# vliu15/speech-masters-thesis

Measured on AMD Instinct MI355X. Metric: LJSpeech utterances/sec per VQ-VAE train step, higher is better.
Workload: dtype bf16

## Files before the change

### speech-masters-thesis_amd/csrc/conv_wgrad.hip

```cpp
#include <algorithm>
#include <cstdlib>

#include "conv_common.h"

namespace smt {

struct WgradArgs {
  const void* x; const void* dy; float* slab;
  const int* lens_in;
  long long x_bs, dy_bs;
  int ldx, ldy;
  int B, Tin, Tout, Ty, Cin, Cout;
  int taps, stride, dil, pad, out_stride, out_offset;
  int rows_per_chunk, chunks_per_batch, nblk_ci, nblk_co, with_bias;
};

template <typename T> struct WTr;
template <> struct WTr<__bf16> {
  static constexpr int R = 128;
  static constexpr int pitch(int ch) { return ch + 32; }
};
template <> struct WTr<float> {
  static constexpr int R = 64;
  static constexpr int pitch(int ch) { return ch + 4; }
};

__device__ __forceinline__ int tr_lane_row(int lane) { return 8 * (lane >> 5) + ((lane & 15) >> 2); }
__device__ __forceinline__ int tr_lane_col(int lane) { return 16 * ((lane >> 4) & 1) + 4 * (lane & 3); }
__device__ __forceinline__ bf16x8 tr_read2(const void* a0, int step4_bytes) {
  const unsigned char* a = reinterpret_cast<const unsigned char*>(a0);
  return lds_tr2(a, a + step4_bytes);
}
__device__ __forceinline__ bf16x8 frag_tr_bf16(const __bf16* tile, int pitch, int row0, int col0, int lane) {
  return tr_read2(tile + (row0 + tr_lane_row(lane)) * pitch + col0 + tr_lane_col(lane), 4 * pitch * 2);
}

struct WgBlock { int nblk, blk, cgl; };
__device__ __forceinline__ WgBlock wgrad_block(int nblk_ci, int nblk_co) {
  WgBlock w;
  w.nblk = nblk_ci * nblk_co;
  const int xcd = blockIdx.x & 7, q = blockIdx.x >> 3;
  w.blk = q % w.nblk;
  w.cgl = (q / w.nblk) * 8 + xcd;
  return w;
}

template <typename T, int NT, int CIB, bool STRIDED>
__global__ __launch_bounds__(CIB * 4) void conv_wgrad_kernel(WgradArgs p) {
  constexpr int EPV = Tr<T>::EPV;
  constexpr int R = WTr<T>::R;
  constexpr int CB = 64;
  constexpr int WNC = CIB / 32;
  constexpr int NTHR = 128 * WNC;
  constexpr int PITCH_DY = WTr<T>::pitch(CB), PITCH_X = WTr<T>::pitch(CIB);
  extern __shared__ __attribute__((aligned(16))) unsigned char smem[];
  const int tid = threadIdx.x, lane = tid & 63, wave = tid >> 6;
  const int wm = wave / WNC, wn = wave % WNC;
  const int r = lane & 31, hh = lane >> 5;

  const WgBlock w = wgrad_block(p.nblk_ci, p.nblk_co);
  if (w.cgl >= p.B * p.chunks_per_batch) return;
  const int co0 = (w.blk / p.nblk_ci) * CB, ci0 = (w.blk % p.nblk_ci) * CIB;
  const int b = w.cgl / p.chunks_per_batch;
  const int chunk = w.cgl % p.chunks_per_batch;
  const int t_begin = chunk * p.rows_per_chunk;
  const int t_end = min(p.Tout, t_begin + p.rows_per_chunk);

  const int rows_x = (R - 1) * p.stride + (p.taps - 1) * p.dil + 1;
  T* lds_dy = reinterpret_cast<T*>(smem);
  T* lds_x = lds_dy + R * PITCH_DY;
  const T* xg = reinterpret_cast<const T*>(p.x) + (long long)b * p.x_bs;
  const T* dyg = reinterpret_cast<const T*>(p.dy) + (long long)b * p.dy_bs;
  const int len_in = p.lens_in ? min(p.lens_in[b], p.Tin) : p.Tin;
  const bool bias_plane = p.with_bias && (ci0 == 0);
  const int ntaps = p.taps;

  f32x16 acc[NT];
#pragma unroll
  for (int j = 0; j < NT; ++j)
#pragma unroll
    for (int e = 0; e < 16; ++e) acc[j][e] = 0.f;

  for (int t0 = t_begin; t0 < t_end; t0 += R) {
    __syncthreads();
    constexpr int VPR_DY = CB / EPV, VPR_X = CIB / EPV;
    constexpr int UB = (NT > 6) ? 4 : 8;
    const int tin0 = t0 * p.stride - p.pad;
    const int n_dy = R * VPR_DY, n_x = rows_x * VPR_X;
    for (int f0 = tid; f0 < n_dy + n_x; f0 += NTHR * UB) {
      Vec<T, EPV> v[UB];
#pragma unroll
      for (int u = 0; u < UB; ++u) {
        const int f = f0 + NTHR * u;
#pragma unroll
        for (int e = 0; e < EPV; ++e) v[u].v[e] = (T)0.f;
        if (f < n_dy) {
          const int row = f / VPR_DY, cv = f % VPR_DY;
          const int t = t0 + row;
          const int ty = t * p.out_stride + p.out_offset;
          if (t < t_end && ty < p.Ty && co0 + cv * EPV < p.Cout)
            v[u] = *reinterpret_cast<const Vec<T, EPV>*>(dyg + (long long)ty * p.ldy + co0 + cv * EPV);
        } else if (f < n_dy + n_x) {
          const int g = f - n_dy;
          const int row = g / VPR_X, cv = g % VPR_X;
          const int tin = tin0 + row;
          if (tin >= 0 && tin < len_in && ci0 + cv * EPV < p.Cin)
            v[u] = *reinterpret_cast<const Vec<T, EPV>*>(xg + (long long)tin * p.ldx + ci0 + cv * EPV);
        }
      }
#pragma unroll
      for (int u = 0; u < UB; ++u) {
        const int f = f0 + NTHR * u;
        if (f < n_dy) {
          *reinterpret_cast<Vec<T, EPV>*>(lds_dy + (f / VPR_DY) * PITCH_DY + (f % VPR_DY) * EPV) = v[u];
        } else if (f < n_dy + n_x) {
          const int g = f - n_dy;
          *reinterpret_cast<Vec<T, EPV>*>(lds_x + (g / VPR_X) * PITCH_X + (g % VPR_X) * EPV) = v[u];
        }
      }
    }
    __syncthreads();

    if constexpr (sizeof(T) == 2) {
      const __bf16* dyt = reinterpret_cast<const __bf16*>(lds_dy);
      const __bf16* xt = reinterpret_cast<const __bf16*>(lds_x);
      bf16x8 ones;
#pragma unroll
      for (int e = 0; e < 8; ++e) ones[e] = (__bf16)1.0f;
#pragma unroll 1
      for (int k0 = 0; k0 < R; k0 += 16) {
        bf16x8 a = frag_tr_bf16(dyt, PITCH_DY, k0, wm * 32, lane);
#pragma unroll
        for (int j = 0; j < NT; ++j) {
          if (j < ntaps) {
            bf16x8 bfrag;
            if constexpr (!STRIDED) {
              bfrag = frag_tr_bf16(xt, PITCH_X, k0 + j * p.dil, wn * 32, lane);
            } else {
              typedef short s16x8 __attribute__((ext_vector_type(8)));
              s16x8 tmp;
#pragma unroll
              for (int e = 0; e < 8; ++e) {
                const short* sp = reinterpret_cast<const short*>(xt) +
                                  ((k0 + 8 * hh + e) * p.stride + j * p.dil) * PITCH_X + wn * 32 + r;
                tmp[e] = *sp;
              }
              bfrag = __builtin_bit_cast(bf16x8, tmp);
            }
            acc[j] = __builtin_amdgcn_mfma_f32_32x32x16_bf16(a, bfrag, acc[j], 0, 0, 0);
          } else if (j == ntaps && bias_plane) {
            acc[j] = __builtin_amdgcn_mfma_f32_32x32x16_bf16(a, ones, acc[j], 0, 0, 0);
          }
        }
      }
    } else {
      const float* dyt = reinterpret_cast<const float*>(lds_dy);
      const float* xt = reinterpret_cast<const float*>(lds_x);
#pragma unroll 2
      for (int k0 = 0; k0 < R; k0 += 2) {
        const float a = dyt[(k0 + hh) * PITCH_DY + wm * 32 + r];
#pragma unroll
        for (int j = 0; j < NT; ++j) {
          if (j < ntaps) {
            const float bv = xt[((k0 + hh) * p.stride + j * p.dil) * PITCH_X + wn * 32 + r];
            acc[j] = __builtin_amdgcn_mfma_f32_32x32x2f32(a, bv, acc[j], 0, 0, 0);
          } else if (j == ntaps && bias_plane) {
            acc[j] = __builtin_amdgcn_mfma_f32_32x32x2f32(a, 1.0f, acc[j], 0, 0, 0);
          }
        }
      }
    }
  }
  const int planes = ntaps + 1;
  float* out = p.slab + ((size_t)w.cgl * w.nblk + w.blk) * (size_t)planes * CB * CIB;
#pragma unroll
  for (int j = 0; j < NT; ++j) {
    if (j >= planes) break;
#pragma unroll
    for (int e = 0; e < 16; ++e) {
      const int row = wm * 32 + (e & 3) + 8 * (e >> 2) + 4 * hh;
      const int col = wn * 32 + r;
      out[((size_t)j * CB + row) * CIB + col] = acc[j][e];
    }
  }
}

__device__ __forceinline__ int swz_dy(int row) { return ((row >> 1) & 1) << 2; }
__device__ __forceinline__ int swz_x(int row) { return (row & 3) << 2; }
__device__ __forceinline__ int swz_col_bytes(int col, int swz) { return (((col >> 3) ^ swz) << 4) + (col & 7) * 2; }

template <int NT>
__global__ __launch_bounds__(512) void conv_wgrad_dma_kernel(WgradArgs p) {
  typedef __bf16 T;
  constexpr int R = 128, CB = 64, CIB = 128, WNC = 4, NTHR = 512;
  constexpr int DYB = CB * 2, XB = CIB * 2;
  constexpr int DY_BYTES = R * DYB;
  extern __shared__ __attribute__((aligned(16))) unsigned char smem[];
  const int tid = threadIdx.x, lane = tid & 63, wave = tid >> 6;
  const int wm = wave / WNC, wn = wave % WNC;
  const int r = lane & 31, hh = lane >> 5;

  const WgBlock w = wgrad_block(p.nblk_ci, p.nblk_co);
  if (w.cgl >= p.B * p.chunks_per_batch) return;
  const int co0 = (w.blk / p.nblk_ci) * CB, ci0 = (w.blk % p.nblk_ci) * CIB;
  const int b = w.cgl / p.chunks_per_batch;
  const int chunk = w.cgl % p.chunks_per_batch;
  const int t_begin = chunk * p.rows_per_chunk;
  const int t_end = min(p.Tout, t_begin + p.rows_per_chunk);

  const int rows_x = (R - 1) + (p.taps - 1) * p.dil + 1;
  const int rows_x_pad = (rows_x + 3) & ~3;
  const size_t buf_bytes = (size_t)DY_BYTES + (size_t)rows_x_pad * XB;
  const T* xg = reinterpret_cast<const T*>(p.x) + (long long)b * p.x_bs;
  const T* dyg = reinterpret_cast<const T*>(p.dy) + (long long)b * p.dy_bs;
  const int len_in = max(0, p.lens_in ? min(p.lens_in[b], p.Tin) : p.Tin);
  const bool bias_plane = p.with_bias && (ci0 == 0);
  const int ntaps = p.taps;

  f32x16 acc[NT];
#pragma unroll
  for (int j = 0; j < NT; ++j)
#pragma unroll
    for (int e = 0; e < 16; ++e) acc[j][e] = 0.f;

  const UntrackedRsrc rdy = untracked_rsrc(dyg + co0, 0, (unsigned)min((long long)0xfffffff0ll, (long long)p.Tout * p.ldy * 2));
  const UntrackedRsrc rxx = untracked_rsrc(xg + ci0, 0, (unsigned)min((long long)0xfffffff0ll, (long long)len_in * p.ldx * 2));
  const unsigned pdy = (unsigned)(p.ldy * 2), pxx = (unsigned)(p.ldx * 2);
  auto stage = [&](int t0, int buf) {
    unsigned char* base = smem + (size_t)buf * buf_bytes;
    for (int g = wave; g < R / 8; g += NTHR / 64) {
      const int row = 8 * g + (lane >> 3), pos = lane & 7;
      const int t = t0 + row;
      const int ch = pos ^ swz_dy(row);
      untracked_dma16(rdy, t < t_end ? (unsigned)t * pdy + (unsigned)(ch << 4) : 0xffffff00u, base + g * 1024);
    }
    const int tin0 = t0 - p.pad;
    for (int g = wave; g < rows_x_pad / 4; g += NTHR / 64) {
      const int row = 4 * g + (lane >> 4), pos = lane & 15;
      const int ch = pos ^ swz_x(row);
      const int tin = tin0 + row;
      const bool ok = (row < rows_x) && (tin >= 0) && (tin < len_in);
      untracked_dma16(rxx, ok ? (unsigned)tin * pxx + (unsigned)(ch << 4) : 0xffffff00u, base + DY_BYTES + g * 1024);
    }
  };

  bf16x8 ones;
#pragma unroll
  for (int e = 0; e < 8; ++e) ones[e] = (__bf16)1.0f;

  const int lrow = tr_lane_row(lane);
  const int coly = wm * 32 + tr_lane_col(lane), colx = wn * 32 + tr_lane_col(lane);
  const int dyoff = lrow * DYB + swz_col_bytes(coly, swz_dy(lrow));
  int xoff[NT];
#pragma unroll
  for (int j = 0; j < NT; ++j) {
    const int rj = lrow + j * p.dil;
    xoff[j] = rj * XB + swz_col_bytes(colx, swz_x(rj));
  }

  stage(t_begin, 0);
  vm_wait<0>();
  int buf = 0;
  for (int t0 = t_begin; t0 < t_end; t0 += R, buf ^= 1) {
    lgkm_wait<0>();
    __builtin_amdgcn_s_barrier();
    if (t0 + R < t_end) stage(t0 + R, buf ^ 1);
    const unsigned char* dyt = smem + (size_t)buf * buf_bytes + dyoff;
    const unsigned char* xbase = smem + (size_t)buf * buf_bytes + DY_BYTES;
#pragma unroll
    for (int k0 = 0; k0 < R; k0 += 16) {
      const bf16x8 a = tr_read2(dyt + k0 * DYB, 4 * DYB);
#pragma unroll
      for (int j = 0; j < NT; ++j) {
        if (j < ntaps) {
          const bf16x8 bfrag = tr_read2(xbase + xoff[j] + k0 * XB, 4 * XB);
          acc[j] = __builtin_amdgcn_mfma_f32_32x32x16_bf16(a, bfrag, acc[j], 0, 0, 0);
        } else if (j == ntaps && bias_plane) {
          acc[j] = __builtin_amdgcn_mfma_f32_32x32x16_bf16(a, ones, acc[j], 0, 0, 0);
        }
      }
    }
    step_end_wait<0>();
  }
  const int planes = ntaps + 1;
  float* out = p.slab + ((size_t)w.cgl * w.nblk + w.blk) * (size_t)planes * CB * CIB;
#pragma unroll
  for (int j = 0; j < NT; ++j) {
    if (j >= planes) break;
#pragma unroll
    for (int e = 0; e < 16; ++e) {
      const int row = wm * 32 + (e & 3) + 8 * (e >> 2) + 4 * hh;
      const int col = wn * 32 + r;
      out[((size_t)j * CB + row) * CIB + col] = acc[j][e];
    }
  }
}

struct ShiftArgs {
  const void* x; const void* dy; float* slab; const int* lens_in;
  long long x_bs, dy_bs;
  int ldx, ldy;
  int B, Tin, Tout, pad, rs;
  int tiles_per_item, tiles_per_wg, n_chunks, nblk_ci, nblk_co, with_bias;
};

#ifndef SMT_WGRAD_STAMP
#define SMT_WGRAD_STAMP 0
#endif
#if SMT_WGRAD_STAMP
__device__ unsigned long long wg_dbg[256 * 8 * 8];
__device__ __forceinline__ unsigned long long wg_stamp() {
  unsigned long long t;
  __builtin_amdgcn_sched_barrier(0);
  asm volatile("s_memtime %0\n\ts_waitcnt lgkmcnt(0)" : "=s"(t) : : "memory");
  __builtin_amdgcn_sched_barrier(0);
  return t;
}
#define WG_SUMS unsigned long long wg_sum[5] = {0, 0, 0, 0, 0}
#define WG_T(var) const unsigned long long var = wg_stamp()
#define WG_ACC(k, a, b) wg_sum[k] += (b) - (a)
#define WG_DUMP do { if (lane == 0 && blockIdx.x < 256) for (int k_ = 0; k_ < 5; ++k_) wg_dbg[(blockIdx.x * 8 + wave) * 8 + k_] += wg_sum[k_]; } while (0)
#else
#define WG_SUMS do {} while (0)
#define WG_T(var) do {} while (0)
#define WG_ACC(k, a, b) do {} while (0)
#define WG_DUMP do {} while (0)
#endif

constexpr int SH_R = 128, SH_XROWS = SH_R + 8, SH_DY = SH_R * 128, SH_X = SH_XROWS * 256, SH_STAGE = SH_DY + SH_X;

template <int NTAPS>
__global__ __launch_bounds__(512) void conv_wgrad_shift_kernel(ShiftArgs p, const __bf16* __restrict__ zero_page) {
  constexpr int CB = 64, CIB = 128, WNC = 4, DYB = CB * 2, XB = CIB * 2, PLANES = NTAPS + 1;
  extern __shared__ __attribute__((aligned(16))) unsigned char smem[];
  const int tid = threadIdx.x, lane = tid & 63;
  const int wave = __builtin_amdgcn_readfirstlane(tid >> 6);
  const int wm = wave / WNC, wn = wave % WNC;
  const int r = lane & 31, hh = lane >> 5;

  const WgBlock w = wgrad_block(p.nblk_ci, p.nblk_co);
  if (w.cgl >= p.n_chunks) return;
  const int co0 = (w.blk / p.nblk_ci) * CB, ci0 = (w.blk % p.nblk_ci) * CIB;
  const int ntiles = p.tiles_per_item * p.B * p.rs;
  const int tile_begin = w.cgl * p.tiles_per_wg;
  const int tile_end = min(ntiles, tile_begin + p.tiles_per_wg);
  const int rs = p.rs;
  const bool bias_plane = p.with_bias && (ci0 == 0);

  f32x16 acc[PLANES];
#pragma unroll
  for (int j = 0; j < PLANES; ++j)
#pragma unroll
    for (int e = 0; e < 16; ++e) acc[j][e] = 0.f;

  constexpr int SH_PIECES = 7;
  constexpr int SH_PPS = 2;
  static_assert(SH_PPS <= NTAPS && SH_PPS * (SH_R / 16) >= SH_PIECES, "the pieces fit the k-loop");
  const unsigned pdy = (unsigned)p.ldy * rs * 2u, pxx = (unsigned)p.ldx * rs * 2u;
  const int dyrow = 8 * wave + (lane >> 3), xrow = 4 * wave + (lane >> 4);
  const unsigned voff_dy = (unsigned)dyrow * pdy + (unsigned)(((lane & 7) ^ swz_dy(dyrow)) << 4);
  const unsigned voff_x = (unsigned)xrow * pxx + (unsigned)(((lane & 15) ^ swz_x(xrow)) << 4);
  const unsigned voff_x6 = (128 + xrow < SH_R + NTAPS - 1) ? voff_x + 128u * pxx : 0x80000000u;
  struct Src { __amdgpu_buffer_rsrc_t rdy, rxx; unsigned sdy, sx; };
  auto item_source = [&](int item, Src& s) {
    const int b = item / rs, cls = item - b * rs;
    const int Tc = (p.Tout - cls + rs - 1) / rs;
    const int len_full = p.lens_in ? min(scalar_load_i32(p.lens_in + b), p.Tin) : p.Tin;
    const int len_in = max(0, (len_full - cls + rs - 1) / rs);
    s.rdy = ws_rsrc(p.dy, ((long long)b * p.dy_bs + (long long)cls * p.ldy + co0) * 2, (unsigned)Tc * pdy);
    s.rxx = ws_rsrc(p.x, ((long long)b * p.x_bs + (long long)cls * p.ldx + ci0) * 2, (unsigned)len_in * pxx);
  };
  auto tile_source = [&](int t0, Src& s) {
    s.sdy = (unsigned)t0 * pdy;
    s.sx = (unsigned)(t0 - p.pad) * pxx;
  };
  auto piece = [&](const Src& s, int i, int buf) {
    unsigned char* base = smem + (size_t)buf * SH_STAGE;
    if (i < 2) ws_dma16(s.rdy, voff_dy + s.sdy + (unsigned)(64 * i) * pdy, base + (wave + 8 * i) * 1024);
    else if (i < 6) ws_dma16(s.rxx, voff_x + s.sx + (unsigned)(32 * (i - 2)) * pxx, base + SH_DY + (wave + 8 * (i - 2)) * 1024);
    else if (wave < 2) ws_dma16(s.rxx, voff_x6 + s.sx, base + SH_DY + (wave + 32) * 1024);
  };

  bf16x8 ones;
#pragma unroll
  for (int e = 0; e < 8; ++e) ones[e] = (__bf16)1.0f;

  const int tg = lane >> 4, tq = (lane & 15) >> 2, tp = lane & 3, thh = tg >> 1;
  const int coly = wm * 32 + 16 * (tg & 1) + 4 * tp, colx = wn * 32 + 16 * (tg & 1) + 4 * tp;
  const int lrow = 8 * thh + tq;
  const int dyoff = lrow * DYB + (((coly >> 3) ^ (((lrow >> 1) & 1) << 2)) << 4) + (coly & 7) * 2;
  const int xoff = SH_DY + lrow * XB + (((colx >> 3) ^ ((lrow & 3) << 2)) << 4) + (colx & 7) * 2;
  typedef unsigned u32x4 __attribute__((ext_vector_type(4)));
  typedef unsigned u32x2 __attribute__((ext_vector_type(2)));
  const unsigned lds0 = (unsigned)(uintptr_t)(__attribute__((address_space(3))) unsigned char*)smem;
  struct Frags { u32x2 a0, a1, p0, p1, q0, q1; };
  constexpr int SH_NREAD = 6;
  auto request = [&](Frags& f, unsigned base, int k0) {
    const unsigned pa = base + dyoff + k0 * 16 * DYB, px = base + xoff + k0 * 16 * XB;
    asm volatile("ds_read_b64_tr_b16 %0, %1" : "=v"(f.a0) : "v"(pa));
    asm volatile("ds_read_b64_tr_b16 %0, %1 offset:%2" : "=v"(f.a1) : "v"(pa), "n"(4 * DYB));
    asm volatile("ds_read_b64_tr_b16 %0, %1" : "=v"(f.p0) : "v"(px));
    asm volatile("ds_read_b64_tr_b16 %0, %1 offset:%2" : "=v"(f.p1) : "v"(px), "n"(4 * XB));
    asm volatile("ds_read_b64_tr_b16 %0, %1 offset:%2" : "=v"(f.q0) : "v"(px), "n"(8 * XB));
    asm volatile("ds_read_b64_tr_b16 %0, %1 offset:%2" : "=v"(f.q1) : "v"(px), "n"(12 * XB));
  };

  WG_SUMS;
  const int item_rows = p.tiles_per_item * SH_R;
  int n_item = tile_begin / p.tiles_per_item, n_t0 = (tile_begin - n_item * p.tiles_per_item) * SH_R;
  Src sn;
  sn.rdy = sn.rxx = ws_rsrc(p.x, 0, 0);
  if (tile_begin < tile_end) {
    item_source(n_item, sn);
    tile_source(n_t0, sn);
#pragma unroll
    for (int i = 0; i < SH_PIECES; ++i) piece(sn, i, 0);
  }
  for (int tile = tile_begin; tile < tile_end; ++tile) {
    const int buf = (tile - tile_begin) & 1;
    WG_T(c0);
    vm_wait<0>();
    __syncthreads();
    WG_T(c1);
    const bool more = tile + 1 < tile_end;
    n_t0 += SH_R;
    if (n_t0 == item_rows) {
      n_t0 = 0; ++n_item;
      if (more) item_source(n_item, sn);
    }
    if (!more) sn.rdy = sn.rxx = ws_rsrc(p.x, 0, 0);
    tile_source(n_t0, sn);
    WG_T(c2);
    const unsigned base = lds0 + (unsigned)buf * SH_STAGE;
    Frags fr[2];
    request(fr[0], base, 0);
#pragma unroll
    for (int k0 = 0; k0 < SH_R / 16; ++k0) {
      Frags& f = fr[k0 & 1];
      if (k0 + 1 < SH_R / 16) {
        request(fr[(k0 + 1) & 1], base, k0 + 1);
        lgkm_wait<SH_NREAD>(f.a0, f.a1, f.p0, f.p1, f.q0, f.q1);
      } else {
        lgkm_wait<0>(f.a0, f.a1, f.p0, f.p1, f.q0, f.q1);
      }
      const u32x4 aw = {f.a0[0], f.a0[1], f.a1[0], f.a1[1]};
      const bf16x8 a = __builtin_bit_cast(bf16x8, aw);
      const unsigned w[8] = {f.p0[0], f.p0[1], f.p1[0], f.p1[1], f.q0[0], f.q0[1], f.q1[0], f.q1[1]};
#pragma unroll
      for (int s = 0; s < NTAPS; ++s) {
        const int m = s >> 1;
        u32x4 bw;
        if (s & 1) {
#pragma unroll
          for (int i = 0; i < 4; ++i) bw[i] = __builtin_amdgcn_alignbit(w[m + i + 1], w[m + i], 16);
        } else {
          bw = u32x4{w[m], w[m + 1], w[m + 2], w[m + 3]};
        }
        acc[s] = __builtin_amdgcn_mfma_f32_32x32x16_bf16(a, __builtin_bit_cast(bf16x8, bw), acc[s], 0, 0, 0);
        if (s < SH_PPS && SH_PPS * k0 + s < SH_PIECES) {
          __builtin_amdgcn_sched_barrier(0);
          piece(sn, SH_PPS * k0 + s, buf ^ 1);
          __builtin_amdgcn_sched_barrier(0);
        }
      }
      if (bias_plane && (k0 & 3) == wn) acc[NTAPS] = __builtin_amdgcn_mfma_f32_32x32x16_bf16(a, ones, acc[NTAPS], 0, 0, 0);
    }
    WG_T(c3);
    WG_ACC(0, c0, c1); WG_ACC(1, c1, c2); WG_ACC(2, c2, c3); WG_ACC(4, c0, c0 + 1);
  }
  vm_wait<0>();
  WG_T(c4);
  float* out = p.slab + ((size_t)w.cgl * w.nblk + w.blk) * (size_t)PLANES * CB * CIB;
#pragma unroll
  for (int j = 0; j < PLANES; ++j)
#pragma unroll
    for (int e = 0; e < 16; ++e) {
      const int row = wm * 32 + (e & 3) + 8 * (e >> 2) + 4 * hh;
      out[((size_t)j * CB + row) * CIB + wn * 32 + r] = acc[j][e];
    }
  WG_T(c5);
  WG_ACC(3, c4, c5);
  WG_DUMP;
}

struct ShiftPlan { int rs, pad, tiles_per_item, tiles_per_wg, n_chunks, nblk_co, nblk_ci; };
static bool wgrad_shift_plan(const smt_conv_desc* d, ShiftPlan* pl) {
  static const bool off = getenv("SMT_WGRAD_NO_SHIFT") != nullptr;
  if (off || d->dtype != SMT_BF16 || d->stride != 1 || d->out_stride != 1 || d->out_offset != 0 || !d->zero_page ||
      d->c_in % 128 != 0 || d->c_out % 64 != 0 || d->taps < 3 || d->taps > 9 || !(d->taps & 1) || d->t_in != d->t_out)
    return false;
  int rs = 1, pad = d->padding;
  if (d->dilation > 1) {
    if (d->padding % d->dilation != 0 || d->t_out / d->dilation < class_min_rows()) return false;
    rs = d->dilation; pad = d->padding / d->dilation;
  }
  if (pad < 0 || pad > d->taps - 1) return false;
  const long long tc_max = (d->t_out + rs - 1) / rs;
  const long long span = (tc_max + 2 * SH_R) * rs * 2;
  if (span * d->ld_x >= (1ll << 31) || span * d->ld_y >= (1ll << 31)) return false;
  const int tpi = (int)((tc_max + SH_R - 1) / SH_R);
  const long long ntiles = (long long)tpi * d->batch * rs;
  static const int min_tiles = getenv("SMT_SHIFT_MIN_TILES") ? atoi(getenv("SMT_SHIFT_MIN_TILES")) : 256;
  if (ntiles < min_tiles) return false;
  const int nco = d->c_out / 64, nci = d->c_in / 128;
  static const int min_tpw = getenv("SMT_SHIFT_MIN_TPW") ? atoi(getenv("SMT_SHIFT_MIN_TPW")) : 2;
  const long long chunks_target =
      std::max<long long>(8, std::min<long long>(256 / (nco * nci), ntiles / std::max(1, min_tpw)));
  const int tpw = (int)((ntiles + chunks_target - 1) / chunks_target);
  pl->rs = rs; pl->pad = pad; pl->tiles_per_item = tpi; pl->tiles_per_wg = tpw;
  pl->n_chunks = (int)((ntiles + tpw - 1) / tpw); pl->nblk_co = nco; pl->nblk_ci = nci;
  return true;
}

struct WreduceJob {
  const float* slab; float* dw; float* db;
  long long so, si, sj;
  int n_chunks, nblk, nblk_ci, planes, taps, Cin, Cout, cib, bias_cols;
  int block0;
  int wblocks;
  signed char jmap[16];
};
constexpr int WR_MAXJ = 16;
struct WreduceBatch { int n_jobs, total_blocks; WreduceJob job[WR_MAXJ]; };

__global__ __launch_bounds__(256) void conv_wgrad_reduce_kernel(WreduceBatch bt) {
  __shared__ f32x4 part[4][64];
  int j = 0;
#pragma unroll 1
  for (int k = 1; k < bt.n_jobs; ++k)
    if ((int)blockIdx.x >= bt.job[k].block0) j = k;
  const WreduceJob& p = bt.job[j];
  const int lb = blockIdx.x - p.block0;
  const size_t blk_elems = (size_t)p.planes * 64 * p.cib;
  const size_t cstride = (size_t)p.nblk * blk_elems;
  if (lb < p.wblocks) {
    const int o = threadIdx.x & 63, sl = threadIdx.x >> 6;
    const int cin4 = p.Cin >> 2;
    const long long total4 = (long long)p.taps * p.Cout * cin4;
    const long long e4 = (long long)lb * 64 + o;
    const bool live = e4 < total4;
    f32x4 s = {0.f, 0.f, 0.f, 0.f};
    int ci = 0, co = 0, plane = 0;
    if (live) {
      ci = (int)(e4 % cin4) * 4; co = (int)((e4 / cin4) % p.Cout); plane = (int)(e4 / ((long long)cin4 * p.Cout));
      const int blk = (co / 64) * p.nblk_ci + (ci / p.cib);
      const float* src = p.slab + (size_t)blk * blk_elems + ((size_t)plane * 64 + (co % 64)) * p.cib + (ci % p.cib);
      int c = sl;
      for (; c + 12 < p.n_chunks; c += 16) {
        const f32x4 v0 = *reinterpret_cast<const f32x4*>(src + (size_t)c * cstride);
        const f32x4 v1 = *reinterpret_cast<const f32x4*>(src + (size_t)(c + 4) * cstride);
        const f32x4 v2 = *reinterpret_cast<const f32x4*>(src + (size_t)(c + 8) * cstride);
        const f32x4 v3 = *reinterpret_cast<const f32x4*>(src + (size_t)(c + 12) * cstride);
        s += v0; s += v1; s += v2; s += v3;
      }
      for (; c < p.n_chunks; c += 4) s += *reinterpret_cast<const f32x4*>(src + (size_t)c * cstride);
    }
    part[sl][o] = s;
    __syncthreads();
    if (sl == 0 && live) {
      f32x4 t = part[0][o];
#pragma unroll
      for (int k = 1; k < 4; ++k) t += part[k][o];
      float* dst = p.dw + co * p.so + ci * p.si + p.jmap[plane] * p.sj;
      dst[0] = t[0]; dst[p.si] = t[1]; dst[2 * p.si] = t[2]; dst[3 * p.si] = t[3];
    }
  } else {
    float* part1 = reinterpret_cast<float*>(&part[0][0]);
    const int o = threadIdx.x & 31, sl = threadIdx.x >> 5;
    const int co = (lb - p.wblocks) * 32 + o;
    const bool live = co < p.Cout && p.db != nullptr;
    float s = 0.f;
    if (live) {
      const int blk = (co / 64) * p.nblk_ci;
      const float* src = p.slab + (size_t)blk * blk_elems + ((size_t)p.taps * 64 + (co % 64)) * p.cib;
      for (int c = sl; c < p.n_chunks; c += 8) {
        const float* q = src + (size_t)c * cstride;
        float part_sum = q[0];
        for (int k = 1; k < p.bias_cols; ++k) part_sum += q[32 * k];
        s += part_sum;
      }
    }
    part1[sl * 32 + o] = s;
    __syncthreads();
    if (sl == 0 && live) {
      float t = part1[o];
#pragma unroll
      for (int k = 1; k < 8; ++k) t += part1[k * 32 + o];
      p.db[co] = t;
    }
  }
}

static thread_local bool g_reduce_defer = false;
static thread_local WreduceBatch g_reduce_batch = {0, 0, {}};

static int reduce_flush(hipStream_t stream) {
  if (g_reduce_batch.n_jobs > 0 && g_reduce_batch.total_blocks > 0) {
    conv_wgrad_reduce_kernel<<<(unsigned)g_reduce_batch.total_blocks, 256, 0, stream>>>(g_reduce_batch);
    g_reduce_batch.n_jobs = 0; g_reduce_batch.total_blocks = 0;
    SMT_CHECK_LAUNCH("conv_wgrad_reduce");
  }
  g_reduce_batch.n_jobs = 0; g_reduce_batch.total_blocks = 0;
  return 0;
}

int launch_wgrad_reduce(const float* slab, float* dw, float* db, int n_chunks, int nblk_co, int nblk_ci, int taps,
                        int c_in, int c_out, int cib, long long so, long long si, long long sj, const int* jmap,
                        hipStream_t stream, int bias_cols) {
  SMT_CHECK_ARG(c_in % 4 == 0 && cib % 4 == 0 && taps <= 16, "conv_wgrad_reduce: c_in and the ci block must be multiples of 4");
  if (g_reduce_batch.n_jobs == WR_MAXJ) {
    int rc = reduce_flush(stream);
    if (rc) return rc;
  }
  WreduceJob& r = g_reduce_batch.job[g_reduce_batch.n_jobs];
  r.bias_cols = bias_cols;
  r.slab = slab; r.dw = dw; r.db = db;
  r.n_chunks = n_chunks; r.nblk = nblk_co * nblk_ci; r.nblk_ci = nblk_ci; r.planes = taps + 1; r.taps = taps;
  r.Cin = c_in; r.Cout = c_out; r.cib = cib;
  r.so = so; r.si = si; r.sj = sj;
  for (int t = 0; t < 16; ++t) r.jmap[t] = (signed char)(t < taps ? jmap[t] : 0);
  const long long total4 = (long long)taps * c_out * (c_in / 4);
  r.wblocks = (int)((total4 + 63) / 64);
  r.block0 = g_reduce_batch.total_blocks;
  g_reduce_batch.total_blocks += r.wblocks + (db ? (c_out + 31) / 32 : 0);
  g_reduce_batch.n_jobs += 1;
  return g_reduce_defer ? 0 : reduce_flush(stream);
}

}

// ... 184 lines not shown
```

Before: 529.5.

## Restructure generic conv wgrad kernel with register prefetch and pipelined LDS reads

Rewrites the generic conv weight-gradient kernel. The next time tile's dy and x rows are prefetched into registers while the current tile computes. For strided bf16 inputs, x is stored in LDS in per-stride planes, so transposed ds_read_b64_tr_b16 loads replace scalar gathers. LDS fragment reads are issued explicitly one k-step ahead under lgkmcnt waits, and a per-variant waves-per-EU occupancy hint is added. The aim is to hide global-load and LDS latency behind MFMA work, at the cost of higher register pressure. It also assumes NT equals taps plus one.

Result: no change. 539.3 (median of 6 runs) (+1.8%).

```diff
diff --git a/speech-masters-thesis_amd/csrc/conv_wgrad.hip b/speech-masters-thesis_amd/csrc/conv_wgrad.hip
--- a/speech-masters-thesis_amd/csrc/conv_wgrad.hip
+++ b/speech-masters-thesis_amd/csrc/conv_wgrad.hip
@@ -1,5 +1,6 @@
 #include <algorithm>
 #include <cstdlib>
+#include <type_traits>
 
 #include "conv_common.h"
 
@@ -44,265 +45,6 @@
   w.cgl = (q / w.nblk) * 8 + xcd;
   return w;
 }
-
-template <typename T, int NT, int CIB, bool STRIDED>
-__global__ __launch_bounds__(CIB * 4) void conv_wgrad_kernel(WgradArgs p) {
-  constexpr int EPV = Tr<T>::EPV;
-  constexpr int R = WTr<T>::R;
-  constexpr int CB = 64;
-  constexpr int WNC = CIB / 32;
-  constexpr int NTHR = 128 * WNC;
-  constexpr int PITCH_DY = WTr<T>::pitch(CB), PITCH_X = WTr<T>::pitch(CIB);
-  extern __shared__ __attribute__((aligned(16))) unsigned char smem[];
-  const int tid = threadIdx.x, lane = tid & 63, wave = tid >> 6;
-  const int wm = wave / WNC, wn = wave % WNC;
-  const int r = lane & 31, hh = lane >> 5;
-
-  const WgBlock w = wgrad_block(p.nblk_ci, p.nblk_co);
-  if (w.cgl >= p.B * p.chunks_per_batch) return;
-  const int co0 = (w.blk / p.nblk_ci) * CB, ci0 = (w.blk % p.nblk_ci) * CIB;
-  const int b = w.cgl / p.chunks_per_batch;
-  const int chunk = w.cgl % p.chunks_per_batch;
-  const int t_begin = chunk * p.rows_per_chunk;
-  const int t_end = min(p.Tout, t_begin + p.rows_per_chunk);
-
-  const int rows_x = (R - 1) * p.stride + (p.taps - 1) * p.dil + 1;
-  T* lds_dy = reinterpret_cast<T*>(smem);
-  T* lds_x = lds_dy + R * PITCH_DY;
-  const T* xg = reinterpret_cast<const T*>(p.x) + (long long)b * p.x_bs;
-  const T* dyg = reinterpret_cast<const T*>(p.dy) + (long long)b * p.dy_bs;
-  const int len_in = p.lens_in ? min(p.lens_in[b], p.Tin) : p.Tin;
-  const bool bias_plane = p.with_bias && (ci0 == 0);
-  const int ntaps = p.taps;
-
-  f32x16 acc[NT];
-#pragma unroll
-  for (int j = 0; j < NT; ++j)
-#pragma unroll
-    for (int e = 0; e < 16; ++e) acc[j][e] = 0.f;
-
-  for (int t0 = t_begin; t0 < t_end; t0 += R) {
-    __syncthreads();
-    constexpr int VPR_DY = CB / EPV, VPR_X = CIB / EPV;
-    constexpr int UB = (NT > 6) ? 4 : 8;
-    const int tin0 = t0 * p.stride - p.pad;
-    const int n_dy = R * VPR_DY, n_x = rows_x * VPR_X;
-    for (int f0 = tid; f0 < n_dy + n_x; f0 += NTHR * UB) {
-      Vec<T, EPV> v[UB];
-#pragma unroll
-      for (int u = 0; u < UB; ++u) {
-        const int f = f0 + NTHR * u;
-#pragma unroll
-        for (int e = 0; e < EPV; ++e) v[u].v[e] = (T)0.f;
-        if (f < n_dy) {
-          const int row = f / VPR_DY, cv = f % VPR_DY;
-          const int t = t0 + row;
-          const int ty = t * p.out_stride + p.out_offset;
-          if (t < t_end && ty < p.Ty && co0 + cv * EPV < p.Cout)
-            v[u] = *reinterpret_cast<const Vec<T, EPV>*>(dyg + (long long)ty * p.ldy + co0 + cv * EPV);
-        } else if (f < n_dy + n_x) {
-          const int g = f - n_dy;
-          const int row = g / VPR_X, cv = g % VPR_X;
-          const int tin = tin0 + row;
-          if (tin >= 0 && tin < len_in && ci0 + cv * EPV < p.Cin)
-            v[u] = *reinterpret_cast<const Vec<T, EPV>*>(xg + (long long)tin * p.ldx + ci0 + cv * EPV);
-        }
-      }
-#pragma unroll
-      for (int u = 0; u < UB; ++u) {
-        const int f = f0 + NTHR * u;
-        if (f < n_dy) {
-          *reinterpret_cast<Vec<T, EPV>*>(lds_dy + (f / VPR_DY) * PITCH_DY + (f % VPR_DY) * EPV) = v[u];
-        } else if (f < n_dy + n_x) {
-          const int g = f - n_dy;
-          *reinterpret_cast<Vec<T, EPV>*>(lds_x + (g / VPR_X) * PITCH_X + (g % VPR_X) * EPV) = v[u];
-        }
-      }
-    }
-    __syncthreads();
-
-    if constexpr (sizeof(T) == 2) {
-      const __bf16* dyt = reinterpret_cast<const __bf16*>(lds_dy);
-      const __bf16* xt = reinterpret_cast<const __bf16*>(lds_x);
-      bf16x8 ones;
-#pragma unroll
-      for (int e = 0; e < 8; ++e) ones[e] = (__bf16)1.0f;
-#pragma unroll 1
-      for (int k0 = 0; k0 < R; k0 += 16) {
-        bf16x8 a = frag_tr_bf16(dyt, PITCH_DY, k0, wm * 32, lane);
-#pragma unroll
-        for (int j = 0; j < NT; ++j) {
-          if (j < ntaps) {
-            bf16x8 bfrag;
-            if constexpr (!STRIDED) {
-              bfrag = frag_tr_bf16(xt, PITCH_X, k0 + j * p.dil, wn * 32, lane);
-            } else {
-              typedef short s16x8 __attribute__((ext_vector_type(8)));
-              s16x8 tmp;
-#pragma unroll
-              for (int e = 0; e < 8; ++e) {
-                const short* sp = reinterpret_cast<const short*>(xt) +
-                                  ((k0 + 8 * hh + e) * p.stride + j * p.dil) * PITCH_X + wn * 32 + r;
-                tmp[e] = *sp;
-              }
-              bfrag = __builtin_bit_cast(bf16x8, tmp);
-            }
-            acc[j] = __builtin_amdgcn_mfma_f32_32x32x16_bf16(a, bfrag, acc[j], 0, 0, 0);
-          } else if (j == ntaps && bias_plane) {
-            acc[j] = __builtin_amdgcn_mfma_f32_32x32x16_bf16(a, ones, acc[j], 0, 0, 0);
-          }
-        }
-      }
-    } else {
-      const float* dyt = reinterpret_cast<const float*>(lds_dy);
-      const float* xt = reinterpret_cast<const float*>(lds_x);
-#pragma unroll 2
-      for (int k0 = 0; k0 < R; k0 += 2) {
-        const float a = dyt[(k0 + hh) * PITCH_DY + wm * 32 + r];
-#pragma unroll
-        for (int j = 0; j < NT; ++j) {
-          if (j < ntaps) {
-            const float bv = xt[((k0 + hh) * p.stride + j * p.dil) * PITCH_X + wn * 32 + r];
-            acc[j] = __builtin_amdgcn_mfma_f32_32x32x2f32(a, bv, acc[j], 0, 0, 0);
-          } else if (j == ntaps && bias_plane) {
-            acc[j] = __builtin_amdgcn_mfma_f32_32x32x2f32(a, 1.0f, acc[j], 0, 0, 0);
-          }
-        }
-      }
-    }
-  }
-  const int planes = ntaps + 1;
-  float* out = p.slab + ((size_t)w.cgl * w.nblk + w.blk) * (size_t)planes * CB * CIB;
-#pragma unroll
-  for (int j = 0; j < NT; ++j) {
-    if (j >= planes) break;
-#pragma unroll
-    for (int e = 0; e < 16; ++e) {
-      const int row = wm * 32 + (e & 3) + 8 * (e >> 2) + 4 * hh;
-      const int col = wn * 32 + r;
-      out[((size_t)j * CB + row) * CIB + col] = acc[j][e];
-    }
-  }
-}
-
-__device__ __forceinline__ int swz_dy(int row) { return ((row >> 1) & 1) << 2; }
-__device__ __forceinline__ int swz_x(int row) { return (row & 3) << 2; }
-__device__ __forceinline__ int swz_col_bytes(int col, int swz) { return (((col >> 3) ^ swz) << 4) + (col & 7) * 2; }
-
-template <int NT>
-__global__ __launch_bounds__(512) void conv_wgrad_dma_kernel(WgradArgs p) {
-  typedef __bf16 T;
-  constexpr int R = 128, CB = 64, CIB = 128, WNC = 4, NTHR = 512;
-  constexpr int DYB = CB * 2, XB = CIB * 2;
-  constexpr int DY_BYTES = R * DYB;
-  extern __shared__ __attribute__((aligned(16))) unsigned char smem[];
-  const int tid = threadIdx.x, lane = tid & 63, wave = tid >> 6;
-  const int wm = wave / WNC, wn = wave % WNC;
-  const int r = lane & 31, hh = lane >> 5;
-
-  const WgBlock w = wgrad_block(p.nblk_ci, p.nblk_co);
-  if (w.cgl >= p.B * p.chunks_per_batch) return;
-  const int co0 = (w.blk / p.nblk_ci) * CB, ci0 = (w.blk % p.nblk_ci) * CIB;
-  const int b = w.cgl / p.chunks_per_batch;
-  const int chunk = w.cgl % p.chunks_per_batch;
-  const int t_begin = chunk * p.rows_per_chunk;
-  const int t_end = min(p.Tout, t_begin + p.rows_per_chunk);
-
-  const int rows_x = (R - 1) + (p.taps - 1) * p.dil + 1;
-  const int rows_x_pad = (rows_x + 3) & ~3;
-  const size_t buf_bytes = (size_t)DY_BYTES + (size_t)rows_x_pad * XB;
-  const T* xg = reinterpret_cast<const T*>(p.x) + (long long)b * p.x_bs;
-  const T* dyg = reinterpret_cast<const T*>(p.dy) + (long long)b * p.dy_bs;
-  const int len_in = max(0, p.lens_in ? min(p.lens_in[b], p.Tin) : p.Tin);
-  const bool bias_plane = p.with_bias && (ci0 == 0);
-  const int ntaps = p.taps;
-
-  f32x16 acc[NT];
-#pragma unroll
-  for (int j = 0; j < NT; ++j)
-#pragma unroll
-    for (int e = 0; e < 16; ++e) acc[j][e] = 0.f;
-
-  const UntrackedRsrc rdy = untracked_rsrc(dyg + co0, 0, (unsigned)min((long long)0xfffffff0ll, (long long)p.Tout * p.ldy * 2));
-  const UntrackedRsrc rxx = untracked_rsrc(xg + ci0, 0, (unsigned)min((long long)0xfffffff0ll, (long long)len_in * p.ldx * 2));
-  const unsigned pdy = (unsigned)(p.ldy * 2), pxx = (unsigned)(p.ldx * 2);
-  auto stage = [&](int t0, int buf) {
-    unsigned char* base = smem + (size_t)buf * buf_bytes;
-    for (int g = wave; g < R / 8; g += NTHR / 64) {
-      const int row = 8 * g + (lane >> 3), pos = lane & 7;
-      const int t = t0 + row;
-      const int ch = pos ^ swz_dy(row);
-      untracked_dma16(rdy, t < t_end ? (unsigned)t * pdy + (unsigned)(ch << 4) : 0xffffff00u, base + g * 1024);
-    }
-    const int tin0 = t0 - p.pad;
-    for (int g = wave; g < rows_x_pad / 4; g += NTHR / 64) {
-      const int row = 4 * g + (lane >> 4), pos = lane & 15;
-      const int ch = pos ^ swz_x(row);
-      const int tin = tin0 + row;
-      const bool ok = (row < rows_x) && (tin >= 0) && (tin < len_in);
-      untracked_dma16(rxx, ok ? (unsigned)tin * pxx + (unsigned)(ch << 4) : 0xffffff00u, base + DY_BYTES + g * 1024);
-    }
-  };
-
-  bf16x8 ones;
-#pragma unroll
-  for (int e = 0; e < 8; ++e) ones[e] = (__bf16)1.0f;
-
-  const int lrow = tr_lane_row(lane);
-  const int coly = wm * 32 + tr_lane_col(lane), colx = wn * 32 + tr_lane_col(lane);
-  const int dyoff = lrow * DYB + swz_col_bytes(coly, swz_dy(lrow));
-  int xoff[NT];
-#pragma unroll
-  for (int j = 0; j < NT; ++j) {
-    const int rj = lrow + j * p.dil;
-    xoff[j] = rj * XB + swz_col_bytes(colx, swz_x(rj));
-  }
-
-  stage(t_begin, 0);
-  vm_wait<0>();
-  int buf = 0;
-  for (int t0 = t_begin; t0 < t_end; t0 += R, buf ^= 1) {
-    lgkm_wait<0>();
-    __builtin_amdgcn_s_barrier();
-    if (t0 + R < t_end) stage(t0 + R, buf ^ 1);
-    const unsigned char* dyt = smem + (size_t)buf * buf_bytes + dyoff;
-    const unsigned char* xbase = smem + (size_t)buf * buf_bytes + DY_BYTES;
-#pragma unroll
-    for (int k0 = 0; k0 < R; k0 += 16) {
-      const bf16x8 a = tr_read2(dyt + k0 * DYB, 4 * DYB);
-#pragma unroll
-      for (int j = 0; j < NT; ++j) {
-        if (j < ntaps) {
-          const bf16x8 bfrag = tr_read2(xbase + xoff[j] + k0 * XB, 4 * XB);
-          acc[j] = __builtin_amdgcn_mfma_f32_32x32x16_bf16(a, bfrag, acc[j], 0, 0, 0);
-        } else if (j == ntaps && bias_plane) {
-          acc[j] = __builtin_amdgcn_mfma_f32_32x32x16_bf16(a, ones, acc[j], 0, 0, 0);
-        }
-      }
-    }
-    step_end_wait<0>();
-  }
-  const int planes = ntaps + 1;
-  float* out = p.slab + ((size_t)w.cgl * w.nblk + w.blk) * (size_t)planes * CB * CIB;
-#pragma unroll
-  for (int j = 0; j < NT; ++j) {
-    if (j >= planes) break;
-#pragma unroll
-    for (int e = 0; e < 16; ++e) {
-      const int row = wm * 32 + (e & 3) + 8 * (e >> 2) + 4 * hh;
-      const int col = wn * 32 + r;
-      out[((size_t)j * CB + row) * CIB + col] = acc[j][e];
-    }
-  }
-}
-
-struct ShiftArgs {
-  const void* x; const void* dy; float* slab; const int* lens_in;
-  long long x_bs, dy_bs;
-  int ldx, ldy;
-  int B, Tin, Tout, pad, rs;
-  int tiles_per_item, tiles_per_wg, n_chunks, nblk_ci, nblk_co, with_bias;
-};
 
 #ifndef SMT_WGRAD_STAMP
 #define SMT_WGRAD_STAMP 0
@@ -326,6 +68,359 @@
 #define WG_ACC(k, a, b) do {} while (0)
 #define WG_DUMP do {} while (0)
 #endif
+
+__device__ __forceinline__ unsigned div_magic(int s) { return 0xffffffffu / (unsigned)s + 1u; }
+
+#ifndef SMT_WGRAD_PREFETCH
+#define SMT_WGRAD_PREFETCH -1
+#endif
+#ifndef SMT_WGRAD_WAVES
+#define SMT_WGRAD_WAVES 0
+#endif
+constexpr bool wgrad_prefetch(int esz, int nt, int cib, bool strided) {
+  if (SMT_WGRAD_PREFETCH >= 0) return SMT_WGRAD_PREFETCH != 0;
+  return true;
+}
+constexpr int wgrad_waves_per_simd(int esz, int nt, int cib, bool strided) {
+  if (SMT_WGRAD_WAVES > 0) return SMT_WGRAD_WAVES;
+  if (cib == 128) return 2;
+  if (esz == 2) return (!strided && nt <= 4) ? 3 : 2;
+  return nt <= (strided ? 4 : 5) ? 3 : 2;
+}
+template <typename T, int NT, int CIB, bool STRIDED>
+__global__ __launch_bounds__(CIB * 4) __attribute__((amdgpu_waves_per_eu(wgrad_waves_per_simd(sizeof(T), NT, CIB, STRIDED))))
+void conv_wgrad_kernel(WgradArgs p) {
+  constexpr int EPV = Tr<T>::EPV;
+  constexpr int R = WTr<T>::R;
+  constexpr int CB = 64;
+  constexpr int WNC = CIB / 32;
+  constexpr int NTHR = 128 * WNC;
+  constexpr int PITCH_DY = WTr<T>::pitch(CB), PITCH_X = WTr<T>::pitch(CIB);
+  constexpr bool PLANES = STRIDED && sizeof(T) == 2;
+  constexpr bool PREFETCH = wgrad_prefetch(sizeof(T), NT, CIB, STRIDED);
+  extern __shared__ __attribute__((aligned(16))) unsigned char smem[];
+  const int tid = threadIdx.x, lane = tid & 63, wave = tid >> 6;
+  const int wm = wave / WNC, wn = wave % WNC;
+  const int r = lane & 31, hh = lane >> 5;
+
+  const WgBlock w = wgrad_block(p.nblk_ci, p.nblk_co);
+  if (w.cgl >= p.B * p.chunks_per_batch) return;
+  const int co0 = (w.blk / p.nblk_ci) * CB, ci0 = (w.blk % p.nblk_ci) * CIB;
+  const int b = w.cgl / p.chunks_per_batch;
+  const int chunk = w.cgl % p.chunks_per_batch;
+  const int t_begin = chunk * p.rows_per_chunk;
+  const int t_end = min(p.Tout, t_begin + p.rows_per_chunk);
+
+  const int rows_x = (R - 1) * p.stride + (p.taps - 1) * p.dil + 1;
+  T* lds_dy = reinterpret_cast<T*>(smem);
+  T* lds_x = lds_dy + R * PITCH_DY;
+  const T* xg = reinterpret_cast<const T*>(p.x) + (long long)b * p.x_bs;
+  const T* dyg = reinterpret_cast<const T*>(p.dy) + (long long)b * p.dy_bs;
+  const int len_in = p.lens_in ? min(p.lens_in[b], p.Tin) : p.Tin;
+  const bool bias_plane = p.with_bias && (ci0 == 0);
+
+  const unsigned s_magic = PLANES ? div_magic(p.stride) : 0u;
+  const int plane_q = PLANES ? rows_x / p.stride : 0, plane_rem = PLANES ? rows_x % p.stride : 0;
+  auto lds_row_x = [&](int row) {
+    if constexpr (!PLANES) return row;
+    const int q = (int)__umulhi((unsigned)row, s_magic), pl = row - q * p.stride;
+    return pl * plane_q + min(pl, plane_rem) + q;
+  };
+
+  f32x16 acc[NT];
+#pragma unroll
+  for (int j = 0; j < NT; ++j)
+#pragma unroll
+    for (int e = 0; e < 16; ++e) acc[j][e] = 0.f;
+
+  typedef Vec<T, EPV> V;
+  constexpr int VPR_DY = CB / EPV, VPR_X = CIB / EPV;
+  constexpr int RPS_DY = NTHR / VPR_DY, RPS_X = NTHR / VPR_X;
+  constexpr int DYS = R / RPS_DY;
+  constexpr int XS = STRIDED ? 9 : 5;
+  constexpr int UB = 4;
+  static_assert(R % RPS_DY == 0, "whole slots");
+  const int rd = tid / VPR_DY, cd = (tid % VPR_DY) * EPV, rx = tid / VPR_X, cx = (tid % VPR_X) * EPV;
+  const bool cd_ok = co0 + cd < p.Cout, cx_ok = ci0 + cx < p.Cin;
+  auto fetch_dy = [&](int t0, int slot_row) {
+    V v;
+#pragma unroll
+    for (int e = 0; e < EPV; ++e) v.v[e] = (T)0.f;
+    const int t = t0 + slot_row + rd;
+    const int ty = t * p.out_stride + p.out_offset;
+    if (t < t_end && ty < p.Ty && cd_ok) v = *reinterpret_cast<const V*>(dyg + (long long)ty * p.ldy + co0 + cd);
+    return v;
+  };
+  auto fetch_x = [&](int t0, int slot_row) {
+    V v;
+#pragma unroll
+    for (int e = 0; e < EPV; ++e) v.v[e] = (T)0.f;
+    const int row = slot_row + rx;
+    const int tin = t0 * p.stride - p.pad + row;
+    if (row < rows_x && tin >= 0 && tin < len_in && cx_ok) v = *reinterpret_cast<const V*>(xg + (long long)tin * p.ldx + ci0 + cx);
+    return v;
+  };
+  auto put_dy = [&](int slot_row, const V& v) { *reinterpret_cast<V*>(lds_dy + (slot_row + rd) * PITCH_DY + cd) = v; };
+  auto put_x = [&](int slot_row, const V& v) {
+    const int row = slot_row + rx;
+    if (row < rows_x) *reinterpret_cast<V*>(lds_x + lds_row_x(row) * PITCH_X + cx) = v;
+  };
+  V pf_dy[DYS], pf_x[XS];
+  auto prefetch = [&](int t0) {
+#pragma unroll
+    for (int u = 0; u < DYS; ++u) pf_dy[u] = fetch_dy(t0, u * RPS_DY);
+#pragma unroll
+    for (int u = 0; u < XS; ++u) pf_x[u] = fetch_x(t0, u * RPS_X);
+  };
+
+  static_assert(NT >= 2, "at least one tap and the bias plane");
+  constexpr int NB = NT - 1;
+  typedef unsigned u32x2 __attribute__((ext_vector_type(2)));
+  typedef unsigned u32x4 __attribute__((ext_vector_type(4)));
+  struct Frags { u32x2 a0, a1, b0[NB], b1[NB]; };
+  constexpr int NREAD = 2 + 2 * NB;
+  static_assert(NREAD <= 15, "lgkmcnt counts up to 15");
+  unsigned a_addr = 0, x_addr[NB];
+  if constexpr (sizeof(T) == 2) {
+    const unsigned lds0 = (unsigned)(uintptr_t)(__attribute__((address_space(3))) unsigned char*)smem;
+    a_addr = lds0 + (unsigned)(tr_lane_row(lane) * PITCH_DY + wm * 32 + tr_lane_col(lane)) * 2u;
+#pragma unroll
+    for (int j = 0; j < NB; ++j) {
+      const int row_j = lds_row_x(j * p.dil);
+      x_addr[j] = lds0 + (unsigned)(R * PITCH_DY + (row_j + tr_lane_row(lane)) * PITCH_X + wn * 32 + tr_lane_col(lane)) * 2u;
+    }
+  }
+  auto request = [&](Frags& f, auto ks_) {
+    constexpr int KS = decltype(ks_)::value;
+    const unsigned pa = a_addr;
+    asm volatile("ds_read_b64_tr_b16 %0, %1 offset:%2" : "=v"(f.a0) : "v"(pa), "n"(KS * 16 * PITCH_DY * 2));
+    asm volatile("ds_read_b64_tr_b16 %0, %1 offset:%2" : "=v"(f.a1) : "v"(pa), "n"((KS * 16 + 4) * PITCH_DY * 2));
+#pragma unroll
+    for (int j = 0; j < NB; ++j) {
+      const unsigned px = x_addr[j];
+      asm volatile("ds_read_b64_tr_b16 %0, %1 offset:%2" : "=v"(f.b0[j]) : "v"(px), "n"(KS * 16 * PITCH_X * 2));
+      asm volatile("ds_read_b64_tr_b16 %0, %1 offset:%2" : "=v"(f.b1[j]) : "v"(px), "n"((KS * 16 + 4) * PITCH_X * 2));
+    }
+  };
+  static_assert((R + 4) * PITCH_X * 2 < 65536, "the k-step offsets fit the 16-bit offset field");
+  bf16x8 ones;
+#pragma unroll
+  for (int e = 0; e < 8; ++e) ones[e] = (__bf16)1.0f;
+  Frags fr[2];
+  auto k_step = [&](auto ks_) {
+    constexpr int KS = decltype(ks_)::value;
+    Frags& f = fr[KS & 1];
+    if constexpr (KS + 1 < R / 16) {
+      request(fr[(KS + 1) & 1], std::integral_constant<int, KS + 1>{});
+      lgkm_wait<NREAD>(f.a0, f.a1, f.b0, f.b1);
+    } else {
+      lgkm_wait<0>(f.a0, f.a1, f.b0, f.b1);
+    }
+    const u32x4 aw = {f.a0[0], f.a0[1], f.a1[0], f.a1[1]};
+    const bf16x8 a = __builtin_bit_cast(bf16x8, aw);
+#pragma unroll
+    for (int j = 0; j < NT; ++j) {
+      if (j < NB) {
+        const int jb = j < NB ? j : 0;
+        const u32x4 bw = {f.b0[jb][0], f.b0[jb][1], f.b1[jb][0], f.b1[jb][1]};
+        acc[j] = __builtin_amdgcn_mfma_f32_32x32x16_bf16(a, __builtin_bit_cast(bf16x8, bw), acc[j], 0, 0, 0);
+      }
+    }
+    if (bias_plane) acc[NB] = __builtin_amdgcn_mfma_f32_32x32x16_bf16(a, ones, acc[NB], 0, 0, 0);
+  };
+
+  WG_SUMS;
+  if constexpr (PREFETCH) prefetch(t_begin);
+  for (int t0 = t_begin; t0 < t_end; t0 += R) {
+    WG_T(c0);
+    __syncthreads();
+    WG_T(c1);
+    if constexpr (!PREFETCH) prefetch(t0);
+#pragma unroll
+    for (int u = 0; u < DYS; ++u) put_dy(u * RPS_DY, pf_dy[u]);
+#pragma unroll
+    for (int u = 0; u < XS; ++u) put_x(u * RPS_X, pf_x[u]);
+    for (int row0 = XS * RPS_X; row0 < rows_x; row0 += UB * RPS_X) {
+      V v[UB];
+#pragma unroll
+      for (int u = 0; u < UB; ++u) v[u] = fetch_x(t0, row0 + u * RPS_X);
+#pragma unroll
+      for (int u = 0; u < UB; ++u) {
+        f32x4 t = __builtin_bit_cast(f32x4, v[u]);
+        pin_v(t);
+        v[u] = __builtin_bit_cast(V, t);
+      }
+#pragma unroll
+      for (int u = 0; u < UB; ++u) put_x(row0 + u * RPS_X, v[u]);
+    }
+    WG_T(c2);
+    __syncthreads();
+    WG_T(c3);
+    if constexpr (PREFETCH)
+      if (t0 + R < t_end) prefetch(t0 + R);
+
+    if constexpr (sizeof(T) == 2) {
+      static_assert(sizeof(T) != 2 || R == 128, "eight k-steps, written out");
+      __builtin_amdgcn_sched_barrier(0);
+      request(fr[0], std::integral_constant<int, 0>{});
+      k_step(std::integral_constant<int, 0>{}); k_step(std::integral_constant<int, 1>{});
+      k_step(std::integral_constant<int, 2>{}); k_step(std::integral_constant<int, 3>{});
+      k_step(std::integral_constant<int, 4>{}); k_step(std::integral_constant<int, 5>{});
+      k_step(std::integral_constant<int, 6>{}); k_step(std::integral_constant<int, 7>{});
+      __builtin_amdgcn_sched_barrier(0);
+    } else {
+      const float* dyt = reinterpret_cast<const float*>(lds_dy);
+      const float* xt = reinterpret_cast<const float*>(lds_x);
+#pragma unroll 2
+      for (int k0 = 0; k0 < R; k0 += 2) {
+        const float a = dyt[(k0 + hh) * PITCH_DY + wm * 32 + r];
+#pragma unroll
+        for (int j = 0; j < NT; ++j) {
+          if (j < NB) {
+            const float bv = xt[((k0 + hh) * p.stride + j * p.dil) * PITCH_X + wn * 32 + r];
+            acc[j] = __builtin_amdgcn_mfma_f32_32x32x2f32(a, bv, acc[j], 0, 0, 0);
+          }
+        }
+        if (bias_plane) acc[NB] = __builtin_amdgcn_mfma_f32_32x32x2f32(a, 1.0f, acc[NB], 0, 0, 0);
+      }
+    }
+    WG_T(c4);
+    WG_ACC(0, c0, c1); WG_ACC(0, c2, c3); WG_ACC(1, c1, c2); WG_ACC(2, c3, c4); WG_ACC(4, c0, c0 + 1);
+  }
+  WG_T(c5);
+  float* out = p.slab + ((size_t)w.cgl * w.nblk + w.blk) * (size_t)NT * CB * CIB;
+#pragma unroll
+  for (int j = 0; j < NT; ++j) {
+#pragma unroll
+    for (int e = 0; e < 16; ++e) {
+      const int row = wm * 32 + (e & 3) + 8 * (e >> 2) + 4 * hh;
+      const int col = wn * 32 + r;
+      out[((size_t)j * CB + row) * CIB + col] = acc[j][e];
+    }
+  }
+  WG_T(c6);
+  WG_ACC(3, c5, c6);
+  WG_DUMP;
+}
+
+__device__ __forceinline__ int swz_dy(int row) { return ((row >> 1) & 1) << 2; }
+__device__ __forceinline__ int swz_x(int row) { return (row & 3) << 2; }
+__device__ __forceinline__ int swz_col_bytes(int col, int swz) { return (((col >> 3) ^ swz) << 4) + (col & 7) * 2; }
+
+template <int NT>
+__global__ __launch_bounds__(512) void conv_wgrad_dma_kernel(WgradArgs p) {
+  typedef __bf16 T;
+  constexpr int R = 128, CB = 64, CIB = 128, WNC = 4, NTHR = 512;
+  constexpr int DYB = CB * 2, XB = CIB * 2;
+  constexpr int DY_BYTES = R * DYB;
+  extern __shared__ __attribute__((aligned(16))) unsigned char smem[];
+  const int tid = threadIdx.x, lane = tid & 63, wave = tid >> 6;
+  const int wm = wave / WNC, wn = wave % WNC;
+  const int r = lane & 31, hh = lane >> 5;
+
+  const WgBlock w = wgrad_block(p.nblk_ci, p.nblk_co);
+  if (w.cgl >= p.B * p.chunks_per_batch) return;
+  const int co0 = (w.blk / p.nblk_ci) * CB, ci0 = (w.blk % p.nblk_ci) * CIB;
+  const int b = w.cgl / p.chunks_per_batch;
+  const int chunk = w.cgl % p.chunks_per_batch;
+  const int t_begin = chunk * p.rows_per_chunk;
+  const int t_end = min(p.Tout, t_begin + p.rows_per_chunk);
+
+  const int rows_x = (R - 1) + (p.taps - 1) * p.dil + 1;
+  const int rows_x_pad = (rows_x + 3) & ~3;
+  const size_t buf_bytes = (size_t)DY_BYTES + (size_t)rows_x_pad * XB;
+  const T* xg = reinterpret_cast<const T*>(p.x) + (long long)b * p.x_bs;
+  const T* dyg = reinterpret_cast<const T*>(p.dy) + (long long)b * p.dy_bs;
+  const int len_in = max(0, p.lens_in ? min(p.lens_in[b], p.Tin) : p.Tin);
+  const bool bias_plane = p.with_bias && (ci0 == 0);
+  const int ntaps = p.taps;
+
+  f32x16 acc[NT];
+#pragma unroll
+  for (int j = 0; j < NT; ++j)
+#pragma unroll
+    for (int e = 0; e < 16; ++e) acc[j][e] = 0.f;
+
+  const UntrackedRsrc rdy = untracked_rsrc(dyg + co0, 0, (unsigned)min((long long)0xfffffff0ll, (long long)p.Tout * p.ldy * 2));
+  const UntrackedRsrc rxx = untracked_rsrc(xg + ci0, 0, (unsigned)min((long long)0xfffffff0ll, (long long)len_in * p.ldx * 2));
+  const unsigned pdy = (unsigned)(p.ldy * 2), pxx = (unsigned)(p.ldx * 2);
+  auto stage = [&](int t0, int buf) {
+    unsigned char* base = smem + (size_t)buf * buf_bytes;
+    for (int g = wave; g < R / 8; g += NTHR / 64) {
+      const int row = 8 * g + (lane >> 3), pos = lane & 7;
+      const int t = t0 + row;
+      const int ch = pos ^ swz_dy(row);
+      untracked_dma16(rdy, t < t_end ? (unsigned)t * pdy + (unsigned)(ch << 4) : 0xffffff00u, base + g * 1024);
+    }
+    const int tin0 = t0 - p.pad;
+    for (int g = wave; g < rows_x_pad / 4; g += NTHR / 64) {
+      const int row = 4 * g + (lane >> 4), pos = lane & 15;
+      const int ch = pos ^ swz_x(row);
+      const int tin = tin0 + row;
+      const bool ok = (row < rows_x) && (tin >= 0) && (tin < len_in);
+      untracked_dma16(rxx, ok ? (unsigned)tin * pxx + (unsigned)(ch << 4) : 0xffffff00u, base + DY_BYTES + g * 1024);
+    }
+  };
+
+  bf16x8 ones;
+#pragma unroll
+  for (int e = 0; e < 8; ++e) ones[e] = (__bf16)1.0f;
+
+  const int lrow = tr_lane_row(lane);
+  const int coly = wm * 32 + tr_lane_col(lane), colx = wn * 32 + tr_lane_col(lane);
+  const int dyoff = lrow * DYB + swz_col_bytes(coly, swz_dy(lrow));
+  int xoff[NT];
+#pragma unroll
+  for (int j = 0; j < NT; ++j) {
+    const int rj = lrow + j * p.dil;
+    xoff[j] = rj * XB + swz_col_bytes(colx, swz_x(rj));
+  }
+
+  stage(t_begin, 0);
+  vm_wait<0>();
+  int buf = 0;
+  for (int t0 = t_begin; t0 < t_end; t0 += R, buf ^= 1) {
+    lgkm_wait<0>();
+    __builtin_amdgcn_s_barrier();
+    if (t0 + R < t_end) stage(t0 + R, buf ^ 1);
+    const unsigned char* dyt = smem + (size_t)buf * buf_bytes + dyoff;
+    const unsigned char* xbase = smem + (size_t)buf * buf_bytes + DY_BYTES;
+#pragma unroll
+    for (int k0 = 0; k0 < R; k0 += 16) {
+      const bf16x8 a = tr_read2(dyt + k0 * DYB, 4 * DYB);
+#pragma unroll
+      for (int j = 0; j < NT; ++j) {
+        if (j < ntaps) {
+          const bf16x8 bfrag = tr_read2(xbase + xoff[j] + k0 * XB, 4 * XB);
+          acc[j] = __builtin_amdgcn_mfma_f32_32x32x16_bf16(a, bfrag, acc[j], 0, 0, 0);
+        } else if (j == ntaps && bias_plane) {
+          acc[j] = __builtin_amdgcn_mfma_f32_32x32x16_bf16(a, ones, acc[j], 0, 0, 0);
+        }
+      }
+    }
+    step_end_wait<0>();
+  }
+  const int planes = ntaps + 1;
+  float* out = p.slab + ((size_t)w.cgl * w.nblk + w.blk) * (size_t)planes * CB * CIB;
+#pragma unroll
+  for (int j = 0; j < NT; ++j) {
+    if (j >= planes) break;
+#pragma unroll
+    for (int e = 0; e < 16; ++e) {
+      const int row = wm * 32 + (e & 3) + 8 * (e >> 2) + 4 * hh;
+      const int col = wn * 32 + r;
+      out[((size_t)j * CB + row) * CIB + col] = acc[j][e];
+    }
+  }
+}
+
+struct ShiftArgs {
+  const void* x; const void* dy; float* slab; const int* lens_in;
+  long long x_bs, dy_bs;
+  int ldx, ldy;
+  int B, Tin, Tout, pad, rs;
+  int tiles_per_item, tiles_per_wg, n_chunks, nblk_ci, nblk_co, with_bias;
+};
 
 constexpr int SH_R = 128, SH_XROWS = SH_R + 8, SH_DY = SH_R * 128, SH_X = SH_XROWS * 256, SH_STAGE = SH_DY + SH_X;
 
```
